# chansoopark98/Deep-Visual-SLAM

Measured on AMD Instinct MI355X. Metric: VO training-step frames/sec (3-frame 640x480 snippets), higher is better.
Workload: dtype f32; 1 GPU; configs[2]/[3]: full 4-scale photometric+smoothness loss, batch 12 per GPU, ResNet-18; per_gpu_batch=12, global_batch=12, num_scales=4, image=640x480, parallelism=dp1, streams=depth | pose | 2x weight-gradient, optimizer=fused Adam pass at lr 0: every step computes from the seeded weights, gpu_max_hw_queues=4

## Files before the change

deep-visual-slam_amd/csrc/conv_dma.h:

```cpp
#pragma once

__device__ __attribute__((aligned(16))) float g_dvs_zero_page[4] = {0.f, 0.f, 0.f, 0.f};

__device__ __forceinline__ void dma16(const float* gp, float* lds_wave_base) {
    __builtin_amdgcn_global_load_lds((const __attribute__((address_space(1))) void*)gp,
                                     (__attribute__((address_space(3))) void*)lds_wave_base, 16, 0, 0);
}

template <int TM, int TN>
__device__ __forceinline__ void mfma_stage_swz(const float* __restrict__ As, const float* __restrict__ Bs, int a_row0,
                                               int b_row0, int lane, f32x16 (&acc)[TM][TN]) {
    const int r = lane & 31, h = lane >> 5;
#pragma unroll
    for (int j = 0; j < BK / 8; ++j) {
        f32x4 a[TM], b[TN];
#pragma unroll
        for (int m = 0; m < TM; ++m) {
            int row = a_row0 + m * 32 + r;
            a[m] = *reinterpret_cast<const f32x4*>(As + row * BK + (((2 * j + h) ^ ((row >> 1) & 7)) << 2));
        }
#pragma unroll
        for (int n = 0; n < TN; ++n) {
            int row = b_row0 + n * 32 + r;
            b[n] = *reinterpret_cast<const f32x4*>(Bs + row * BK + (((2 * j + h) ^ ((row >> 1) & 7)) << 2));
        }
#pragma unroll
        for (int t = 0; t < 4; ++t)
#pragma unroll
            for (int m = 0; m < TM; ++m)
#pragma unroll
                for (int n = 0; n < TN; ++n)
                    acc[m][n] = __builtin_amdgcn_mfma_f32_32x32x2f32(a[m][t], b[n][t], acc[m][n], 0, 0, 0);
    }
}

template <int I, int N, class F>
__device__ __forceinline__ void static_for(F&& f) {
    if constexpr (I < N) {
        f(std::integral_constant<int, I>{});
        static_for<I + 1, N>(f);
    }
}

template <int BM, int BN, int WM, int WN, int MODE>
__global__ __launch_bounds__(NT) void conv_dma_kernel(FwdParams p) {
    constexpr int TM = BM / WM / 32, TN = BN / WN / 32;
    constexpr int A_INS = BM / 32, B_INS = BN / 32;
    constexpr int MAXTAP = 9;
    static_assert(WM * WN == 4 && TM >= 1 && TN >= 1, "4 waves");
    extern __shared__ __attribute__((aligned(16))) float smem[];
    float* As = smem;
    float* Bs = smem + 2 * BM * BK;

    ConvShape s = p.s;
    const int tid = threadIdx.x, lane = tid & 63;
    const int wave = __builtin_amdgcn_readfirstlane(tid >> 6);
    const int wm = wave / WN, wn = wave % WN;
    int bid_x, bid_y, bid_z, ks = 0;
    if (p.g.z > 1) {
        int lg = blockIdx.x;
        bid_x = lg % p.g.x;
        lg /= p.g.x;
        bid_y = lg % p.g.y;
        bid_z = lg / p.g.y;
    } else {
        const int tiles = p.g.x * p.g.y;
        int lg = blockIdx.x;
        if (p.ksplit > 1) {
            ks = lg % p.ksplit;
            lg /= p.ksplit;
        }
        lg = xcd_logical(lg, tiles, p.ksplit > 1 ? 0 : p.g.remap);
        bid_y = lg % p.g.y;
        bid_x = lg / p.g.y;
        bid_z = 0;
    }
    const int m0 = bid_x * BM, n0 = bid_y * BN;

    int Hr = s.Ho, Wr = s.Wo, rstep = 1, oy0 = 0, ox0 = 0, ky0 = 0, kx0 = 0;
    if (MODE == IN_DGRAD && s.stride == 2) {
        const int py = bid_z >> 1, px = bid_z & 1;
        oy0 = (py - s.pad) & 1;
        ox0 = (px - s.pad) & 1;
        Hr = (s.Ho - oy0 + 1) >> 1;
        Wr = (s.Wo - ox0 + 1) >> 1;
        rstep = 2;
        ky0 = py;
        kx0 = px;
        s.kh = py < s.kh ? (s.kh - py + 1) >> 1 : 0;
        s.kw = px < s.kw ? (s.kw - px + 1) >> 1 : 0;
        s.Ktot = s.kh * s.kw * s.Cin;
    }
    const int M = s.B * Hr * Wr;
    if (m0 >= M) return;
    const int ntap = s.kh * s.kw, nC = s.Cin / BK;
    const int c_per = (nC + p.ksplit - 1) / max(p.ksplit, 1);
    const int c_lo = p.ksplit > 1 ? ks * c_per : 0, c_hi = p.ksplit > 1 ? min(nC, c_lo + c_per) : nC;

    constexpr int NO_TAP = OOB_OFF;
    const int rsub = lane >> 3, slot = lane & 7;
    int toff[A_INS][MAXTAP];
    int toff2[(MODE == IN_UPCAT) ? A_INS : 1][MAXTAP];
    int r_b[A_INS], r_y[A_INS], r_x[A_INS], r_q[A_INS];
    bool r_ok[A_INS];
#pragma unroll
    for (int j = 0; j < A_INS; ++j) {
        const int row = (wave * A_INS + j) * 8 + rsub;
        r_q[j] = (slot ^ ((row >> 1) & 7)) << 2;
        int m = m0 + row;
        r_ok[j] = m < M;
        m = min(m, M - 1);
        const int b = m / (Hr * Wr), rem = m - b * (Hr * Wr);
        const int oy = rem / Wr, ox = rem - oy * Wr;
        r_b[j] = b;
        if (MODE == IN_DGRAD) {
            r_y[j] = oy * rstep + oy0 + s.pad;
            r_x[j] = ox * rstep + ox0 + s.pad;
        } else {
            r_y[j] = oy * s.stride - s.pad;
            r_x[j] = ox * s.stride - s.pad;
        }
    }
    int kc_tap[MAXTAP];
#pragma unroll
    for (int t = 0; t < MAXTAP; ++t) {
        kc_tap[t] = 0;
#pragma unroll
        for (int j = 0; j < A_INS; ++j) {
            toff[j][t] = NO_TAP;
            if (MODE == IN_UPCAT) toff2[j][t] = NO_TAP;
        }
        if (t < ntap) {
            const int tky = (t >= s.kw ? 1 : 0) + (t >= 2 * s.kw ? 1 : 0), tkx = t - tky * s.kw;
            kc_tap[t] = (MODE == IN_DGRAD) ? ((ky0 + rstep * tky) * p.s.kw + (kx0 + rstep * tkx)) * s.Cin : t * s.Cin;
#pragma unroll
            for (int j = 0; j < A_INS; ++j) {
                bool ok = r_ok[j];
                int off = 0, off2 = 0;
                if (MODE == IN_DGRAD) dgrad_tap_setup(p.s, r_b[j], r_y[j], r_x[j], ky0 + rstep * tky, kx0 + rstep * tkx, ok, off);
                else tap_setup<MODE>(s, p.t, r_b[j], r_y[j] + tky, r_x[j] + tkx, ok, off, off2);
                toff[j][t] = ok ? (off + r_q[j]) * 4 : NO_TAP;
                if (MODE == IN_UPCAT) toff2[j][t] = ok ? (off2 + p.t.C1 + r_q[j]) * 4 : NO_TAP;
            }
        }
    }
    int b_off[B_INS];
#pragma unroll
    for (int j = 0; j < B_INS; ++j) {
        const int row = (wave * B_INS + j) * 8 + rsub;
        const int n = n0 + row;
        b_off[j] = (n < s.Cout) ? (n * p.s.Ktot + ((slot ^ ((row >> 1) & 7)) << 2)) * 4 : NO_TAP;
    }
    const size_t x_elems = (MODE == IN_UPCAT) ? (size_t)s.B * (s.H >> 1) * (s.W >> 1) * p.t.C1 : (size_t)s.B * s.H * s.W * s.Cin;
    const __amdgpu_buffer_rsrc_t rx = dma_rsrc(p.x, x_elems * 4);
    const __amdgpu_buffer_rsrc_t rx2 = (MODE == IN_UPCAT && p.t.x2 != p.x)
                                           ? dma_rsrc(p.t.x2, (size_t)s.B * s.H * s.W * (s.Cin - p.t.C1) * 4) : rx;
    const __amdgpu_buffer_rsrc_t rw = dma_rsrc(p.w, (size_t)p.s.Cout * p.s.Ktot * 4);

    auto issue = [&](auto tc, int c, int buf) {
        constexpr int T = decltype(tc)::value;
        const int ci0 = c * BK;
        if (MODE == IN_UPCAT && ci0 >= p.t.C1) {
            const int soff = (ci0 - p.t.C1) * 4;
#pragma unroll
            for (int j = 0; j < A_INS; ++j) dma16_buf(rx2, toff2[j][T], soff, As + (buf * BM + (wave * A_INS + j) * 8) * BK);
        } else {
            const int soff = ci0 * 4;
#pragma unroll
            for (int j = 0; j < A_INS; ++j) dma16_buf(rx, toff[j][T], soff, As + (buf * BM + (wave * A_INS + j) * 8) * BK);
        }
        const int kc = (kc_tap[T] + ci0) * 4;
#pragma unroll
        for (int j = 0; j < B_INS; ++j) dma16_buf(rw, b_off[j], kc, Bs + (buf * BN + (wave * B_INS + j) * 8) * BK);
    };

    f32x16 acc[TM][TN];
#pragma unroll
    for (int m = 0; m < TM; ++m)
#pragma unroll
        for (int n = 0; n < TN; ++n)
#pragma unroll
            for (int i = 0; i < 16; ++i) acc[m][n][i] = 0.f;

    int buf = 0;
    auto compute_and_sync = [&]() {
        mfma_stage_swz<TM, TN>(As + buf * BM * BK, Bs + buf * BN * BK, wm * TM * 32, wn * TN * 32, lane, acc);
        asm volatile("s_waitcnt vmcnt(0)" ::: "memory");
        __syncthreads();
        buf ^= 1;
    };
    if (ntap > 0) {
        issue(std::integral_constant<int, 0>{}, c_lo, 0);
        asm volatile("s_waitcnt vmcnt(0)" ::: "memory");
        __syncthreads();
    }
    static_for<0, MAXTAP>([&](auto tc) {
        constexpr int T = decltype(tc)::value;
        if (T < ntap) {
#pragma unroll 1
            for (int c = c_lo; c + 1 < c_hi; ++c) {
                issue(tc, c + 1, buf ^ 1);
                compute_and_sync();
            }
            if constexpr (T + 1 < MAXTAP) {
                if (T + 1 < ntap) issue(std::integral_constant<int, T + 1>{}, c_lo, buf ^ 1);
            }
            compute_and_sync();
        }
    });
    int* rowtab = nullptr;
    if (MODE == IN_DGRAD && rstep == 2) {
        rowtab = reinterpret_cast<int*>(smem);
        fill_row_table<BM>(p, s, rowtab, m0, M, Hr, Wr, rstep, oy0, ox0);
    }
    conv_epilogue<TM, TN, MODE>(p, s, acc, m0, n0, wm, wn, lane, M, Hr, Wr, rstep, oy0, ox0, rowtab, BM);
}
```

deep-visual-slam_amd/csrc/conv_fwd.hip:

```cpp
#include "conv_common.h"

#include <cstdlib>
#include <type_traits>

namespace {
using namespace dvsconv;

struct FwdParams {
    const float* x;
    const float* w;
    const float* bias;
    float* y;
    float* stats;
    int stat_split;
    float* y2;
    int split_c1;
    int dbg_nobarrier;
    const float* zero_page;
    const float* res;
    int stat_mask, stat_stride;
    int work_m;
    int ksplit;
    Grid3 g;
    ConvShape s;
// ... 130 lines not shown
        for (int tn = 0; tn < TN; ++tn) {
            const int n = n0 + (wn * TN + tn) * 32 + ln;
#pragma unroll
            for (int tm = 0; tm < TM; ++tm) {
                const int mb = m0 + (wm * TM + tm) * 32 + 4 * lh;
#pragma unroll
                for (int i = 0; i < 16; ++i) {
                    const int m = mb + (i & 3) + 8 * (i >> 2);
                    if (m < M && n < s.Cout) atomicAdd(p.y + (size_t)m * s.Cout + n, acc[tm][tn][i]);
                }
            }
        }
    } else if (stats == 0) {
        if (p.res) conv_epilogue_body<TM, TN, MODE, 0, true, true>(p, s, acc, m0, n0, wm, wn, lane, M, rowtab, bm);
        else if (act) conv_epilogue_body<TM, TN, MODE, 0, true>(p, s, acc, m0, n0, wm, wn, lane, M, rowtab, bm);
        else conv_epilogue_body<TM, TN, MODE, 0, false>(p, s, acc, m0, n0, wm, wn, lane, M, rowtab, bm);
    } else if (stats == 1) {
        if (act) conv_epilogue_body<TM, TN, MODE, 1, true>(p, s, acc, m0, n0, wm, wn, lane, M, rowtab, bm);
        else conv_epilogue_body<TM, TN, MODE, 1, false>(p, s, acc, m0, n0, wm, wn, lane, M, rowtab, bm);
    } else {
        conv_epilogue_body<TM, TN, MODE, 2, true>(p, s, acc, m0, n0, wm, wn, lane, M, rowtab, bm);
    }
}

#include "conv_dma.h"

template <int BM, int BN, int WM, int WN, int MODE, bool FOLD, int NBUF, bool BF16 = false>
__global__ __launch_bounds__(NT) void conv_fwd_kernel(FwdParams p) {
    constexpr int TM = BM / WM / 32, TN = BN / WN / 32;
    constexpr int A_VECS = BM / 32, B_VECS = BN / 32;
    static_assert(WM * WN == 4 && TM >= 1 && TN >= 1, "4 waves");
    extern __shared__ __attribute__((aligned(16))) float smem[];
    float* As = smem;
    float* Bs = smem + NBUF * BM * LDK;
    __bf16* Ah = reinterpret_cast<__bf16*>(smem);
    __bf16* Bh = Ah + NBUF * BM * LDKH;

    ConvShape s = p.s;
    const int tid = threadIdx.x, lane = tid & 63, wave = tid >> 6;
    const int wm = wave / WN, wn = wave % WN;
    int bid_x, bid_y, bid_z;
    if (p.g.z > 1) {
        int lg = blockIdx.x;
        bid_x = lg % p.g.x;
        lg /= p.g.x;
        bid_y = lg % p.g.y;
        bid_z = lg / p.g.y;
    } else {
        int lg = xcd_logical(blockIdx.x, p.g.x * p.g.y, p.g.remap);
        bid_y = lg % p.g.y;
        bid_x = lg / p.g.y;
        bid_z = 0;
    }
    const int m0 = bid_x * BM, n0 = bid_y * BN;
    const int c4 = (tid & 7) * 4, r0 = tid >> 3;

    int Hr = s.Ho, Wr = s.Wo, rstep = 1, oy0 = 0, ox0 = 0, ky0 = 0, kx0 = 0, kw_full = s.kw;
    if (MODE == IN_DGRAD && s.stride == 2) {
        const int py = bid_z >> 1, px = bid_z & 1;
        oy0 = (py - s.pad) & 1;
        ox0 = (px - s.pad) & 1;
        Hr = (s.Ho - oy0 + 1) >> 1;
        Wr = (s.Wo - ox0 + 1) >> 1;
        rstep = 2;
        ky0 = py;
        kx0 = px;
        s.kh = py < s.kh ? (s.kh - py + 1) >> 1 : 0;
        s.kw = px < s.kw ? (s.kw - px + 1) >> 1 : 0;
        s.Ktot = s.kh * s.kw * s.Cin;
    }
    const int M = s.B * Hr * Wr;
    if (m0 >= M) return;

    int a_b[A_VECS], a_iy[A_VECS], a_ix[A_VECS];
    bool a_ok[A_VECS];
#pragma unroll
    for (int j = 0; j < A_VECS; ++j) {
        int m = m0 + r0 + 32 * j;
        a_ok[j] = m < M;
        m = min(m, M - 1);
        int b = m / (Hr * Wr), rem = m - b * (Hr * Wr);
        int oy = rem / Wr, ox = rem - oy * Wr;
        a_b[j] = b;
        if (MODE == IN_DGRAD) {
            a_iy[j] = oy * rstep + oy0 + s.pad;
            a_ix[j] = ox * rstep + ox0 + s.pad;
        } else {
            a_iy[j] = oy * s.stride - s.pad;
            a_ix[j] = ox * s.stride - s.pad;
        }
    }
    const float* b_ptr[B_VECS];
    bool b_ok[B_VECS];
#pragma unroll
    for (int j = 0; j < B_VECS; ++j) {
        int n = n0 + r0 + 32 * j;
        b_ok[j] = n < s.Cout;
        b_ptr[j] = p.w + (size_t)min(n, s.Cout - 1) * p.s.Ktot;
    }

    KPos kp;
    kp.init(c4, s);
    f32x4 ra[A_VECS], rb[B_VECS], ry[A_VECS], re[A_VECS], fsc, fsh;
    bool ra_ok[A_VECS], rb_ok;
    unsigned ra_mask[A_VECS];
    float psc = 1.f, psh = 0.f;
    int t_off[A_VECS], t_off2[A_VECS], cur_tap = -1;
    bool t_ok[A_VECS];
    auto load_stage = [&]() {
        const bool k_ok = kp.k < s.Ktot;
        int kc = min(kp.k, p.s.Ktot - 4);
        const int ky = ky0 + rstep * kp.ky, kx = kx0 + rstep * kp.kx;
        if (MODE == IN_DGRAD) kc = k_ok ? (ky * kw_full + kx) * s.Cin + kp.ci : 0;
        const int tap = ky * kw_full + kx;
        if (MODE != IN_PLANAR && tap != cur_tap) {
            cur_tap = tap;
#pragma unroll
            for (int j = 0; j < A_VECS; ++j) {
                bool ok = a_ok[j];
                if (MODE == IN_DGRAD) dgrad_tap_setup(p.s, a_b[j], a_iy[j], a_ix[j], ky, kx, ok, t_off[j]);
                else tap_setup<MODE>(s, p.t, a_b[j], a_iy[j] + kp.ky, a_ix[j] + kp.kx, ok, t_off[j], t_off2[j]);
                t_ok[j] = ok;
                if (p.dbg_nobarrier & 2) t_off[j] = t_off2[j] = 0;
            }
        }
#pragma unroll
        for (int j = 0; j < A_VECS; ++j) {
            if (MODE == IN_PLANAR) {
                int ci;
                ra[j] = gather_planar_raw(p.x, s, a_b[j], a_iy[j], a_ix[j], kc, a_ok[j] && k_ok, ra_mask[j], ci);
                if (FOLD && j == 0) {
                    psc = p.t.in_scale[ci];
                    psh = p.t.in_shift[ci];
                }
            } else if (MODE == IN_DGRAD) {
                ra[j] = *reinterpret_cast<const f32x4*>(p.x + (t_off[j] + kp.ci));
                if (p.t.dact) ry[j] = *reinterpret_cast<const f32x4*>(p.t.aux + (t_off[j] + kp.ci));
                re[j] = f32x4{0.f, 0.f, 0.f, 0.f};
                if (p.s.pad_mode == PAD_REFLECT)
                    re[j] = dgrad_reflect_extra(p.x, p.s, p.t, a_b[j], a_iy[j], a_ix[j], ky, kx, kp.ci, a_ok[j] && k_ok);
                ra_ok[j] = t_ok[j] && k_ok;
            } else {
                ra[j] = load_tap4<MODE>(p.x, p.t, t_off[j], t_off2[j], kp.ci);
                ra_ok[j] = t_ok[j] && k_ok;
            }
        }
        if (FOLD && MODE != IN_PLANAR) {
            fsc = *reinterpret_cast<const f32x4*>(p.t.in_scale + kp.ci);
            fsh = *reinterpret_cast<const f32x4*>(p.t.in_shift + kp.ci);
        }
#pragma unroll
        for (int j = 0; j < B_VECS; ++j) rb[j] = *reinterpret_cast<const f32x4*>(b_ptr[j] + kc);
        rb_ok = k_ok;
        if (MODE == IN_PLANAR) kp.k += BK;
        else kp.advance(s);
    };
    auto store_stage = [&](int buf) {
#pragma unroll
        for (int j = 0; j < A_VECS; ++j) {
            f32x4 v;
            if (MODE == IN_PLANAR) v = finalize_planar<FOLD>(ra[j], ra_mask[j], psc, psh);
            else if (MODE == IN_DGRAD) v = finalize_dgrad(ra[j], ry[j], re[j], ra_ok[j], p.t.dact);
            else v = finalize<FOLD>(ra[j], ra_ok[j], fsc, fsh, p.t.in_relu);
            if constexpr (BF16) *reinterpret_cast<bf16x4*>(Ah + (buf * BM + r0 + 32 * j) * LDKH + c4) = to_bf16(v);
            else *reinterpret_cast<f32x4*>(As + (buf * BM + r0 + 32 * j) * LDK + c4) = v;
        }
#pragma unroll
        for (int j = 0; j < B_VECS; ++j) {
            const bool ok = b_ok[j] && rb_ok;
            f32x4 v = rb[j];
#pragma unroll
            for (int e = 0; e < 4; ++e) v[e] = ok ? v[e] : 0.f;
            if constexpr (BF16) *reinterpret_cast<bf16x4*>(Bh + (buf * BN + r0 + 32 * j) * LDKH + c4) = to_bf16(v);
            else *reinterpret_cast<f32x4*>(Bs + (buf * BN + r0 + 32 * j) * LDK + c4) = v;
        }
    };

    f32x16 acc[TM][TN];
#pragma unroll
    for (int m = 0; m < TM; ++m)
#pragma unroll
        for (int n = 0; n < TN; ++n)
#pragma unroll
            for (int i = 0; i < 16; ++i) acc[m][n][i] = 0.f;

    const int KT = (s.Ktot + BK - 1) / BK;
    load_stage();
    store_stage(0);
    __syncthreads();
#pragma unroll 1
    for (int kt = 0; kt < KT; ++kt) {
        const int buf = (NBUF == 2) ? (kt & 1) : 0;
        const bool staged = !(p.dbg_nobarrier & 4);
        if (staged && kt + 1 < KT) load_stage();
        if constexpr (BF16) mfma_stage_bf16<TM, TN>(Ah + buf * BM * LDKH, Bh + buf * BN * LDKH, wm * TM * 32, wn * TN * 32, lane, acc);
        else mfma_stage<TM, TN>(As + buf * BM * LDK, Bs + buf * BN * LDK, wm * TM * 32, wn * TN * 32, lane, acc);
        if (NBUF == 1 && !(p.dbg_nobarrier & 1)) __syncthreads();
        if (staged && kt + 1 < KT) store_stage((NBUF == 2) ? (buf ^ 1) : 0);
        if (!(p.dbg_nobarrier & 1)) __syncthreads();
    }

    int* rowtab = nullptr;
    if (MODE == IN_DGRAD && (rstep == 2 || p.split_c1 > 0)) {
        rowtab = reinterpret_cast<int*>(smem);
        fill_row_table<BM>(p, s, rowtab, m0, M, Hr, Wr, rstep, oy0, ox0);
    }
    conv_epilogue<TM, TN, MODE>(p, s, acc, m0, n0, wm, wn, lane, M, Hr, Wr, rstep, oy0, ox0, rowtab, BM);
}

int conv_nbuf() {
    static int v = [] {
        const char* e = getenv("DVS_CONV_NBUF");
        return (e && e[0] == '2') ? 2 : 1;
    }();
    return v;
}

template <int BM, int BN, int WM, int WN, int MODE, bool FOLD, int NBUF, bool BF16 = false>
void launch_buf(const FwdParams& p, hipStream_t st, int slot);

template <int MODE, bool FOLD>
bool dma_eligible(const FwdParams& p) {
    static const bool enabled = [] { const char* e = getenv("DVS_CONV_DMA"); return !(e && e[0] == '0'); }();
    if (!enabled || FOLD || MODE == IN_PLANAR || (p.s.Cin % BK) != 0 || p.s.kh > 3 || p.s.kw > 3) return false;
    const double lim = 2147483648.0 / 4;
    if ((double)p.s.B * p.s.H * p.s.W * p.s.Cin >= lim || (double)p.s.Cout * p.s.Ktot >= lim) return false;
    if (MODE == IN_DGRAD) return p.t.dact == 0 && p.s.pad_mode == PAD_ZERO && p.split_c1 == 0;
    return true;
}

inline int xcd_remap_enabled() {
    static const int on = [] { const char* e = getenv("DVS_CONV_XCD"); return !(e && e[0] == '0') ? 1 : 0; }();
    return on;
}

__global__ __launch_bounds__(256) void splitk_finish_kernel(float* __restrict__ y, const float* __restrict__ bias,
                                                            const float* __restrict__ res, size_t nvec, int cout4, int act) {
    const size_t i = (size_t)blockIdx.x * 256 + threadIdx.x;
    if (i >= nvec) return;
    f32x4 v = reinterpret_cast<f32x4*>(y)[i];
    if (bias) v += reinterpret_cast<const f32x4*>(bias)[i % cout4];
    if (res) v += reinterpret_cast<const f32x4*>(res)[i];
#pragma unroll
    for (int e = 0; e < 4; ++e) v[e] = apply_act(v[e], act);
    reinterpret_cast<f32x4*>(y)[i] = v;
}

__global__ __launch_bounds__(256) void splitk_zero_kernel(float* __restrict__ y, size_t nvec) {
    const size_t i = (size_t)blockIdx.x * 256 + threadIdx.x;
    if (i < nvec) reinterpret_cast<f32x4*>(y)[i] = f32x4{0.f, 0.f, 0.f, 0.f};
}

template <int BM, int BN, int WM, int WN, int MODE>
void launch_dma(const FwdParams& p, hipStream_t st, int slot) {
    int M = p.s.B * p.s.Ho * p.s.Wo;
    dim3 grid((M + BM - 1) / BM, (p.s.Cout + BN - 1) / BN);
    if (MODE == IN_DGRAD && p.s.stride == 2) {
        int mc = p.s.B * ((p.s.Ho + 1) / 2) * ((p.s.Wo + 1) / 2);
        grid = dim3((mc + BM - 1) / BM, (p.s.Cout + BN - 1) / BN, 4);
    }
    size_t lds = (size_t)2 * (BM + BN) * BK * sizeof(float);
    auto kern = conv_dma_kernel<BM, BN, WM, WN, MODE>;
    static bool attr_set = false;
    if (!attr_set && lds > 64 * 1024 - 256) {
        (void)hipFuncSetAttribute(reinterpret_cast<const void*>(kern), hipFuncAttributeMaxDynamicSharedMemorySize, (int)lds);
        attr_set = true;
    }
    dvs::ProfScope prof(slot, st);
    const double eff = (MODE == IN_DGRAD) ? 1.0 / (p.s.stride * p.s.stride) : 1.0;
    prof.work(2.0 * (p.work_m ? p.work_m : M) * p.s.Cout * (double)p.s.Ktot * eff);
    FwdParams q = p;
    q.g = Grid3{(int)grid.x, (int)grid.y, (int)grid.z, xcd_remap_enabled()};
    q.ksplit = 1;
    if (MODE != IN_DGRAD || (p.s.stride == 1 && p.split_c1 == 0)) {
        static const bool splitk = [] { const char* e = getenv("DVS_CONV_SPLITK"); return !(e && e[0] == '0'); }();
        const int tiles = grid.x * grid.y, nC = p.s.Cin / BK;
        static const int sk_tiles = [] { const char* e = getenv("DVS_SPLITK_TILES"); return e ? atoi(e) : 320; }();
        static const int sk_target = [] { const char* e = getenv("DVS_SPLITK_TARGET"); return e ? atoi(e) : 0; }();
        if (splitk && !dvs::deterministic() && !p.stats && tiles < sk_tiles && nC >= 2 && (p.s.Cout & 3) == 0) {
            const int target = sk_target > 0 ? sk_target : (tiles < 200 ? 256 : 1024);
            int want = min(nC, (target + tiles - 1) / tiles);
            const int per = (nC + want - 1) / want;
            q.ksplit = (nC + per - 1) / per;
        }
    }
    static const float* zp = [] {
        void* d = nullptr;
        (void)hipGetSymbolAddress(&d, HIP_SYMBOL(g_dvs_zero_page));
        return static_cast<const float*>(d);
    }();
    q.zero_page = zp;
    if (q.ksplit > 1) {
        const size_t nvec = (size_t)M * p.s.Cout / 4;
        hipLaunchKernelGGL(splitk_zero_kernel, dim3((unsigned)((nvec + 255) / 256)), dim3(256), 0, st, p.y, nvec);
        hipLaunchKernelGGL(kern, dim3(grid.x * grid.y * q.ksplit), dim3(NT), lds, st, q);
        if (p.bias || p.res || p.act != ACT_NONE)
            hipLaunchKernelGGL(splitk_finish_kernel, dim3((unsigned)((nvec + 255) / 256)), dim3(256), 0, st, p.y, p.bias, p.res,
                               nvec, p.s.Cout / 4, p.act);
        return;
    }
    hipLaunchKernelGGL(kern, dim3(grid.x * grid.y * grid.z), dim3(NT), lds, st, q);
}

template <int BM, int BN, int WM, int WN, int MODE, bool FOLD>
void launch_cfg(const FwdParams& p0, hipStream_t st, int slot) {
    FwdParams p = p0;
    if constexpr (MODE == IN_PLANAR) {
        if (dvs::precision_bf16()) {
            p.dbg_nobarrier = 0;
            launch_buf<BM, BN, WM, WN, MODE, FOLD, 2, true>(p, st, slot);
            return;
        }
    }
    if constexpr (!FOLD && MODE != IN_PLANAR) {
        if (dvs::precision_bf16() && (p.s.Cin & 3) == 0) {
            p.dbg_nobarrier = 0;
            launch_buf<BM, BN, WM, WN, MODE, FOLD, 2, true>(p, st, slot);
            return;
        }
        if (dma_eligible<MODE, FOLD>(p)) {
            launch_dma<BM, BN, WM, WN, MODE>(p, st, slot);
            return;
        }
    }
    static const int nobar = dvs::experiment_flags("DVS_CONV_DEBUG_NOBARRIER");
    p.dbg_nobarrier = nobar;
    if (conv_nbuf() == 2) launch_buf<BM, BN, WM, WN, MODE, FOLD, 2>(p, st, slot);
    else launch_buf<BM, BN, WM, WN, MODE, FOLD, 1>(p, st, slot);
}

template <int BM, int BN, int WM, int WN, int MODE, bool FOLD, int NBUF, bool BF16>
void launch_buf(const FwdParams& p, hipStream_t st, int slot) {
    int M = p.s.B * p.s.Ho * p.s.Wo;
    dim3 grid((M + BM - 1) / BM, (p.s.Cout + BN - 1) / BN);
    if (MODE == IN_DGRAD && p.s.stride == 2) {
        int mc = p.s.B * ((p.s.Ho + 1) / 2) * ((p.s.Wo + 1) / 2);
        grid = dim3((mc + BM - 1) / BM, (p.s.Cout + BN - 1) / BN, 4);
    }
    size_t lds = BF16 ? (size_t)NBUF * (BM + BN) * LDKH * 2 : (size_t)NBUF * (BM + BN) * LDK * sizeof(float);
    if (BF16 && MODE == IN_DGRAD && lds < (size_t)2 * BM * sizeof(int)) lds = (size_t)2 * BM * sizeof(int);
    auto kern = conv_fwd_kernel<BM, BN, WM, WN, MODE, FOLD, NBUF, BF16>;
    static bool attr_set = false;
    if (!attr_set && lds > 64 * 1024) {
        (void)hipFuncSetAttribute(reinterpret_cast<const void*>(kern), hipFuncAttributeMaxDynamicSharedMemorySize, (int)lds);
        attr_set = true;
    }
    dvs::ProfScope prof(slot, st);
    const double k_real = (MODE == IN_PLANAR) ? (double)p.s.Cin * p.s.kh * p.s.kw : (double)p.s.Ktot;
    const double eff = (MODE == IN_DGRAD) ? 1.0 / (p.s.stride * p.s.stride) : 1.0;
    prof.work(2.0 * (p.work_m ? p.work_m : M) * p.s.Cout * k_real * eff);
    FwdParams q = p;
    q.g = Grid3{(int)grid.x, (int)grid.y, (int)grid.z, xcd_remap_enabled()};
    hipLaunchKernelGGL(kern, dim3(grid.x * grid.y * grid.z), dim3(NT), lds, st, q);
}

template <int MODE, bool FOLD>
void launch_mode(const FwdParams& p, hipStream_t st, int slot) {
    const ConvShape& s = p.s;
    const int M = s.B * s.Ho * s.Wo;
    static const bool small = [] { const char* e = getenv("DVS_CONV_TILE"); return e && e[0] == 's'; }();
    if constexpr (MODE == IN_DGRAD && !FOLD) {
        static const bool n96 = [] { const char* e = getenv("DVS_CONV_N96"); return !(e && e[0] == '0'); }();
        if (n96 && s.Cout == 96 && (dvs::precision_bf16() || !dma_eligible<MODE, FOLD>(p))) {
            FwdParams q = p;
            q.dbg_nobarrier = 0;
            if (dvs::precision_bf16()) launch_buf<128, 96, 4, 1, MODE, FOLD, 2, true>(q, st, slot);
            else if (conv_nbuf() == 2) launch_buf<128, 96, 4, 1, MODE, FOLD, 2>(q, st, slot);
            else launch_buf<128, 96, 4, 1, MODE, FOLD, 1>(q, st, slot);
            return;
        }
    }
    if (s.Cout > 64) {
        static const bool small_m = [] { const char* e = getenv("DVS_CONV_SMALLM"); return !(e && e[0] == '0'); }();
        const int t64 = ((M + 63) / 64) * ((s.Cout + 127) / 128);
        const int t128 = ((M + 127) / 128) * ((s.Cout + 127) / 128);
        const double rounds = t128 / 512.0, full = ceil(rounds);
        const bool tail_waste = rounds <= 3.2 && (full - rounds) / full > 0.2;
        const bool gemm_small = s.kh == 1 && s.kw == 1 && MODE != IN_DGRAD && t64 < 224;
        if (small_m && MODE != IN_DGRAD && ((p.stats && t64 < 160) || gemm_small)) launch_cfg<64, 64, 2, 2, MODE, FOLD>(p, st, slot);
        else if (small || t128 < 448 || tail_waste) launch_cfg<64, 128, 1, 4, MODE, FOLD>(p, st, slot);
        else launch_cfg<128, 128, 2, 2, MODE, FOLD>(p, st, slot);
    } else if (s.Cout > 32) {
        if (small) launch_cfg<64, 64, 2, 2, MODE, FOLD>(p, st, slot);
        else launch_cfg<128, 64, 2, 2, MODE, FOLD>(p, st, slot);
    } else {
        launch_cfg<128, 32, 4, 1, MODE, FOLD>(p, st, slot);
    }
}

__global__ __launch_bounds__(256) void pack_wt_kernel(const float* __restrict__ w, float* __restrict__ wt, int Cout,
                                                      int Cin, int T) {
    __shared__ float tile[32][33];
    const int tap = blockIdx.z, ci0 = blockIdx.x * 32, co0 = blockIdx.y * 32;
    const int tx = threadIdx.x & 31, ty = threadIdx.x >> 5;
#pragma unroll
    for (int j = 0; j < 4; ++j) {
        int co = co0 + ty + 8 * j, ci = ci0 + tx;
        tile[ty + 8 * j][tx] = (co < Cout && ci < Cin) ? w[((size_t)co * T + tap) * Cin + ci] : 0.f;
    }
    __syncthreads();
#pragma unroll
    for (int j = 0; j < 4; ++j) {
        int ci = ci0 + ty + 8 * j, co = co0 + tx;
        if (ci < Cin && co < Cout) wt[((size_t)ci * T + tap) * Cout + co] = tile[tx][ty + 8 * j];
    }
}

__global__ __launch_bounds__(256) void act_bwd_kernel(const float* __restrict__ dy, const float* __restrict__ y,
                                                      float* __restrict__ dz, size_t nvec, int act, float* __restrict__ dbias,
                                                      int C) {
    __shared__ f32x4 red[256];
    f32x4 bsum = {0.f, 0.f, 0.f, 0.f};
    const size_t stride = (size_t)gridDim.x * 256;
    for (size_t i = (size_t)blockIdx.x * 256 + threadIdx.x; i < nvec; i += stride) {
        f32x4 g = reinterpret_cast<const f32x4*>(dy)[i];
        const f32x4 v = reinterpret_cast<const f32x4*>(y)[i];
        if (act == ACT_ELU) {
#pragma unroll
            for (int e = 0; e < 4; ++e) g[e] = fmaf(g[e], fminf(v[e], 0.f), g[e]);
        } else {
#pragma unroll
            for (int e = 0; e < 4; ++e) g[e] *= act_grad_from_out(v[e], act);
        }
        reinterpret_cast<f32x4*>(dz)[i] = g;
        bsum += g;
    }
    if (dbias) {
        const int cv = C / 4;
        red[threadIdx.x] = bsum;
        __syncthreads();
        if ((int)threadIdx.x < cv) {
            for (int k = threadIdx.x + cv; k < 256; k += cv) bsum += red[k];
#pragma unroll
            for (int e = 0; e < 4; ++e) atomicAdd(dbias + threadIdx.x * 4 + e, bsum[e]);
        }
    }
}

__device__ __forceinline__ f32x4 folded_at(const float* __restrict__ G, int b, int y, int x, int c, int H, int W, int C) {
    const int Wp = W + 2;
    const float* base = G + ((size_t)b * (H + 2)) * Wp * C + c;
    auto at = [&](int py, int px) { return *reinterpret_cast<const f32x4*>(base + ((size_t)py * Wp + px) * C); };
    const int ey = (y == 1) ? 0 : ((y == H - 2) ? H + 1 : -1), ex = (x == 1) ? 0 : ((x == W - 2) ? W + 1 : -1);
    f32x4 v = at(y + 1, x + 1);
    if (ey >= 0) v += at(ey, x + 1);
    if (ex >= 0) v += at(y + 1, ex);
    if (ey >= 0 && ex >= 0) v += at(ey, ex);
    if (H == 3 && y == 1) v += at(H + 1, x + 1) + ((ex >= 0) ? at(H + 1, ex) : f32x4{0.f, 0.f, 0.f, 0.f});
    if (W == 3 && x == 1) v += at(y + 1, W + 1) + ((ey >= 0) ? at(ey, W + 1) : f32x4{0.f, 0.f, 0.f, 0.f});
    if (H == 3 && W == 3 && y == 1 && x == 1) v += at(H + 1, W + 1);
    return v;
}
__global__ __launch_bounds__(256) void reflect_fold_kernel(const float* __restrict__ G, float* __restrict__ dx,
                                                           float* __restrict__ dx_skip, int B, int H, int W, int C, int C1) {
    const int cv = C / 4;
    const size_t i = (size_t)blockIdx.x * 256 + threadIdx.x;
    if (C1 == 0) {
        if (i >= (size_t)B * H * W * cv) return;
        const int c = (int)(i % cv) * 4;
        size_t m = i / cv;
        const int x = (int)(m % W);
        m /= W;
        const int y = (int)(m % H), b = (int)(m / H);
        *reinterpret_cast<f32x4*>(dx + (((size_t)b * H + y) * W + x) * C + c) = folded_at(G, b, y, x, c, H, W, C);
        return;
    }
    const int H2 = H >> 1, W2 = W >> 1;
    if (i >= (size_t)B * H2 * W2 * cv) return;
    const int c = (int)(i % cv) * 4;
    size_t m = i / cv;
    const int x2 = (int)(m % W2);
    m /= W2;
    const int y2 = (int)(m % H2), b = (int)(m / H2);
    f32x4 v[4];
#pragma unroll
    for (int q = 0; q < 4; ++q) v[q] = folded_at(G, b, 2 * y2 + (q >> 1), 2 * x2 + (q & 1), c, H, W, C);
    if (c < C1) {
        *reinterpret_cast<f32x4*>(dx + (((size_t)b * H2 + y2) * W2 + x2) * C1 + c) = (v[0] + v[1]) + (v[2] + v[3]);
    } else {
        const int cs = C - C1;
#pragma unroll
        for (int q = 0; q < 4; ++q)
            *reinterpret_cast<f32x4*>(dx_skip + (((size_t)b * H + 2 * y2 + (q >> 1)) * W + 2 * x2 + (q & 1)) * cs + (c - C1)) = v[q];
    }
}

struct PackEntry {
    const float* w;
    float* wt;
    int Cout, Cin, T, wg_begin;
};
__global__ __launch_bounds__(256) void pack_wt_batch_kernel(const PackEntry* __restrict__ tab, int n) {
    __shared__ float tile[32][33];
    __shared__ int s_e;
    if (threadIdx.x == 0) {
        int e = 0;
        while (e + 1 < n && (int)blockIdx.x >= tab[e + 1].wg_begin) ++e;
        s_e = e;
    }
    __syncthreads();
    const PackEntry en = tab[s_e];
    const int tci = (en.Cin + 31) / 32, tco = (en.Cout + 31) / 32;
    int local = blockIdx.x - en.wg_begin;
    const int tap = local / (tci * tco);
    local -= tap * tci * tco;
    const int co0 = (local / tci) * 32, ci0 = (local % tci) * 32;
    const int tx = threadIdx.x & 31, ty = threadIdx.x >> 5;
#pragma unroll
    for (int j = 0; j < 4; ++j) {
        int co = co0 + ty + 8 * j, ci = ci0 + tx;
        tile[ty + 8 * j][tx] = (co < en.Cout && ci < en.Cin) ? en.w[((size_t)co * en.T + tap) * en.Cin + ci] : 0.f;
    }
    __syncthreads();
#pragma unroll
    for (int j = 0; j < 4; ++j) {
        int ci = ci0 + ty + 8 * j, co = co0 + tx;
        if (ci < en.Cin && co < en.Cout) en.wt[((size_t)ci * en.T + tap) * en.Cout + co] = tile[tx][ty + 8 * j];
    }
}

}

extern "C" {

int dvs_reflect_fold(const float* g_padded, float* dx, float* dx_skip, int B, int H, int W, int C, int C1, void* stream) {
    DVS_REQUIRE(g_padded && dx && B > 0 && H >= 3 && W >= 3 && C > 0 && (C & 3) == 0, "dvs_reflect_fold: bad argument");
    DVS_REQUIRE(C1 == 0 || ((C1 & 3) == 0 && C1 <= C && !((H | W) & 1) && (C1 == C || dx_skip)), "dvs_reflect_fold: bad split");
    const size_t n = (C1 == 0 ? (size_t)B * H * W : (size_t)B * (H / 2) * (W / 2)) * (C / 4);
    hipStream_t st = static_cast<hipStream_t>(stream);
    dvs::ProfScope prof(dvs::SLOT_CONV_DGRAD, st);
    hipLaunchKernelGGL(reflect_fold_kernel, dim3((unsigned)((n + 255) / 256)), dim3(256), 0, st, g_padded, dx, dx_skip, B, H, W, C, C1);
    return dvs::check_launch("dvs_reflect_fold");
}

int dvs_act_bwd(const float* dy, const float* y, float* dz, size_t n, int act, float* dbias, int C, void* stream) {
    DVS_REQUIRE(dy && y && dz && n > 0 && (n & 3) == 0 && act >= 0 && act <= 3, "dvs_act_bwd: bad argument");
    DVS_REQUIRE(!dbias || (C >= 4 && (C & 3) == 0 && C / 4 <= 256 && 256 % (C / 4) == 0 && n % C == 0),
                "dvs_act_bwd: the bias gradient needs C/4 to divide 256 (C=%d)", C);
    const size_t nvec = n / 4;
    size_t blocks = (nvec + 255) / 256;
    if (blocks > 512) blocks = 512;
    if (dbias) {
        size_t few = nvec / (256 * 32);
        few = few < 32 ? 32 : few;
        if (blocks > few) blocks = few;
    }
    hipStream_t st = static_cast<hipStream_t>(stream);
    dvs::ProfScope prof(dvs::SLOT_CONV_DGRAD, st);
    hipLaunchKernelGGL(act_bwd_kernel, dim3((unsigned)blocks), dim3(256), 0, st, dy, y, dz, nvec, act, dbias, C);
    return dvs::check_launch("dvs_act_bwd");
}

int dvs_conv2d_pack_wt_batch(const void* table, int n_entries, int total_workgroups, void* stream) {
    DVS_REQUIRE(table && n_entries > 0 && total_workgroups > 0, "dvs_conv2d_pack_wt_batch: bad argument");
    hipLaunchKernelGGL(pack_wt_batch_kernel, dim3(total_workgroups), dim3(256), 0, static_cast<hipStream_t>(stream),
                       static_cast<const PackEntry*>(table), n_entries);
    return dvs::check_launch("dvs_conv2d_pack_wt_batch");
}

int dvs_conv2d_pack_wt(const float* w, float* wt, int Cout, int Cin, int kh, int kw, void* stream) {
    DVS_REQUIRE(w && wt && Cout > 0 && Cin > 0 && kh > 0 && kw > 0, "dvs_conv2d_pack_wt: bad argument");
    dim3 grid((Cin + 31) / 32, (Cout + 31) / 32, kh * kw);
    hipLaunchKernelGGL(pack_wt_kernel, grid, dim3(256), 0, static_cast<hipStream_t>(stream), w, wt, Cout, Cin, kh * kw);
    return dvs::check_launch("dvs_conv2d_pack_wt");
}

int dvs_conv2d_dgrad(const float* dy, const float* wt, float* dx, const dvs_conv_desc* d, const float* y_out,
                     int dact, float* dx_skip, int C1, void* stream) {
    return dvs_conv2d_dgrad_res(dy, wt, dx, d, y_out, dact, dx_skip, C1, nullptr, stream);
}

int dvs_conv2d_dgrad_res(const float* dy, const float* wt, float* dx, const dvs_conv_desc* d, const float* y_out,
                         int dact, float* dx_skip, int C1, const float* residual, void* stream) {
    DVS_REQUIRE(dy && wt && dx && d, "dvs_conv2d_dgrad: null pointer");
    DVS_REQUIRE(!residual || (C1 == 0 && residual != dx), "dvs_conv2d_dgrad: a residual excludes the upsample+concat split and may not alias dx");
    DVS_REQUIRE(C1 == 0 || (d->stride == 1 && (d->H & 1) == 0 && (d->W & 1) == 0 && C1 <= d->Cin &&
                            (C1 == d->Cin || dx_skip != nullptr)),
                "dvs_conv2d_dgrad: bad upsample+concat split");
    DVS_REQUIRE(d->stride == 1 || d->stride == 2, "dvs_conv2d_dgrad: stride %d (1 or 2 supported)", d->stride);
    DVS_REQUIRE((d->Cout & 3) == 0 && (d->Cin & 3) == 0, "dvs_conv2d_dgrad: channel counts must be multiples of 4");
    DVS_REQUIRE(d->pad_mode == PAD_ZERO || (d->pad_mode == 2 && d->pad == 0 && d->stride == 1 && d->H > 2 && d->W > 2 && !dact && !C1) ||
                    (d->pad_mode == PAD_REFLECT && d->pad == 1 && d->kh == 3 && d->kw == 3 && d->stride == 1 && d->H >= 2 && d->W >= 2),
                "dvs_conv2d_dgrad: reflect mode is ReflectionPad2d(1) + 3x3 stride 1 only; pad_mode 2 = pre-padded input, pad 0");
    DVS_REQUIRE(!dact || y_out, "dvs_conv2d_dgrad: activation gradient needs the forward output");
    DVS_REQUIRE((double)d->B * d->H * d->W * (d->Cin > d->Cout ? d->Cin : d->Cout) < 2147483648.0,
                "dvs_conv2d_dgrad: tensors must have fewer than 2^31 elements (32-bit gather offsets)");
    FwdParams p{};
    p.x = dy; p.w = wt; p.y = dx;
    p.stat_split = 0x7fffffff;
    ConvShape& s = p.s;
    int Ho = (d->H + 2 * d->pad - d->kh) / d->stride + 1, Wo = (d->W + 2 * d->pad - d->kw) / d->stride + 1;
    s.B = d->B;
    s.Ho = d->H; s.Wo = d->W; s.Cout = d->Cin;
    s.H = Ho; s.W = Wo; s.Cin = d->Cout;
    s.kh = d->kh; s.kw = d->kw; s.stride = d->stride; s.pad = d->pad; s.pad_mode = d->pad_mode;
    if (d->pad_mode == 2) {
        s.pad_mode = PAD_ZERO;
        p.work_m = d->B * (d->H - 2) * (d->W - 2);
    }
    s.Ktot = d->kh * d->kw * d->Cout;
    p.t.aux = y_out;
    p.t.dact = dact;
    p.y2 = dx_skip;
    p.split_c1 = C1;
    p.res = residual;
    hipStream_t st = static_cast<hipStream_t>(stream);
    if (!residual && d->pad_mode == PAD_REFLECT && d->kh == 3 && d->kw == 3 && d->stride == 1 && d->pad == 1 &&
        thin_dgrad(dy, wt, dx, y_out, dact, d->B, d->H, d->W, d->Cin, d->Cout, C1, dx_skip, st))
        return dvs::check_launch("dvs_conv2d_dgrad");
    launch_mode<IN_DGRAD, false>(p, st, dvs::SLOT_CONV_DGRAD);
    return dvs::check_launch("dvs_conv2d_dgrad");
}

int dvs_conv2d_fwd(const float* x, const float* w, const float* bias, float* y, const dvs_conv_desc* d,
                   const dvs_conv_fusion* f, void* stream) {
    DVS_REQUIRE(x && w && y && d, "dvs_conv2d_fwd: null pointer");
    DVS_REQUIRE(d->B > 0 && d->H > 0 && d->W > 0 && d->Cin > 0 && d->Cout > 0 && d->kh > 0 && d->kw > 0 &&
                    d->stride > 0 && d->pad >= 0,
                "dvs_conv2d_fwd: bad descriptor");
    FwdParams p{};
    p.x = x; p.w = w; p.bias = bias; p.y = y;
    p.stat_split = 0x7fffffff;
    ConvShape& s = p.s;
    s.B = d->B; s.H = d->H; s.W = d->W; s.Cin = d->Cin; s.Cout = d->Cout;
    s.kh = d->kh; s.kw = d->kw; s.stride = d->stride; s.pad = d->pad; s.pad_mode = d->pad_mode;
    s.Ho = (d->H + 2 * d->pad - d->kh) / d->stride + 1;
    s.Wo = (d->W + 2 * d->pad - d->kw) / d->stride + 1;
    DVS_REQUIRE(s.Ho > 0 && s.Wo > 0, "dvs_conv2d_fwd: empty output");
    DVS_REQUIRE((double)d->B * d->H * d->W * d->Cin < 2147483648.0 && (double)d->B * s.Ho * s.Wo * d->Cout < 2147483648.0,
                "dvs_conv2d_fwd: tensors must have fewer than 2^31 elements (32-bit gather offsets)");
    DVS_REQUIRE(d->pad_mode == PAD_ZERO || (d->pad < d->H && d->pad < d->W), "dvs_conv2d_fwd: reflect pad too large");
    int planar = 0;
    if (f) {
        p.t.x2 = f->x2; p.t.C1 = f->C1; p.t.in_scale = f->in_scale; p.t.in_shift = f->in_shift;
        p.t.in_relu = f->in_relu; planar = f->nchw_planar;
        p.act = f->act; p.stats = f->stats; p.res = f->residual;
        DVS_REQUIRE(f->act >= 0 && f->act <= ACT_GELU, "dvs_conv2d_fwd: unknown activation %d", f->act);
        DVS_REQUIRE(!(f->residual && f->stats), "dvs_conv2d_fwd: residual and stats are exclusive (inference vs training)");
        DVS_REQUIRE(f->stat_groups >= 0 && f->stat_groups <= 2 && (f->stat_groups != 2 || (d->B % 2) == 0),
                    "dvs_conv2d_fwd: stat_groups is 0, 1 or 2 (2 needs an even batch)");
        p.stat_split = (f->stat_groups == 2) ? (d->B / 2) * s.Ho * s.Wo : 0x7fffffff;
        if (f->stats && f->stat_slots > 1) {
            DVS_REQUIRE(f->stat_slots <= 64 && (f->stat_slots & (f->stat_slots - 1)) == 0 && !f->nchw_planar,
                        "dvs_conv2d_fwd: stat_slots must be a power of two <= 64 (NHWC input only)");
            p.stat_mask = f->stat_slots - 1;
            p.stat_stride = (f->stat_groups == 2 ? 2 : 1) * 2 * d->Cout;
        }
        DVS_REQUIRE(!(f->x2) || (f->C1 > 0 && (d->H & 1) == 0 && (d->W & 1) == 0 &&
                                 ((f->C1 == d->Cin && (f->C1 & 3) == 0) || (f->C1 < d->Cin && (f->C1 % BK) == 0))),
                    "dvs_conv2d_fwd: upsample+concat needs C1 %% 32 == 0 (or C1 == Cin) and even H, W");
        DVS_REQUIRE(!(f->x2 && planar), "dvs_conv2d_fwd: planar input cannot be concatenated");
        DVS_REQUIRE((f->in_scale == nullptr) == (f->in_shift == nullptr), "dvs_conv2d_fwd: in_scale/in_shift come together");
    }
    if (planar) {
        DVS_REQUIRE(d->kw <= 8 && d->pad_mode == PAD_ZERO, "dvs_conv2d_fwd: planar input supports kw <= 8, zero padding");
        s.Ktot = d->Cin * d->kh * 8;
    } else {
        DVS_REQUIRE((d->Cin & 3) == 0, "dvs_conv2d_fwd: NHWC input needs Cin %% 4 == 0 (got %d)", d->Cin);
        s.Ktot = d->kh * d->kw * d->Cin;
    }
    hipStream_t st = static_cast<hipStream_t>(stream);
    const bool fold = p.t.in_scale != nullptr;
    static const bool stem16 = [] { const char* e = getenv("DVS_BF16_STEM"); return e && e[0] == '1'; }();
// ... 20 lines not shown
```

Before: 1537 frames/s.

## Merge stride-2 dgrad parity classes into one kernel with shared input tiles

Adds a dedicated stride-2 data-gradient conv kernel that handles all four output parity classes in a single launch. Each loaded gradient tile is reused across the taps of every class, with separate accumulators per class. Stores go through a per-row pixel table held in LDS. Previously the z-grid launched the parity classes as separate blocks that each reloaded the input. The new kernel raises register pressure (four accumulator sets for 3x3) and serializes the classes inside one block, trading parallelism for input reuse.

```diff
diff --git a/deep-visual-slam_amd/csrc/conv_dma.h b/deep-visual-slam_amd/csrc/conv_dma.h
--- a/deep-visual-slam_amd/csrc/conv_dma.h
+++ b/deep-visual-slam_amd/csrc/conv_dma.h
@@ -215,3 +215,177 @@
     }
     conv_epilogue<TM, TN, MODE>(p, s, acc, m0, n0, wm, wn, lane, M, Hr, Wr, rstep, oy0, ox0, rowtab, BM);
 }
+
+template <bool K3>
+struct S2Map {
+    static constexpr int pad = K3 ? 1 : 0;
+    static constexpr int first_shift = K3 ? 0 : 3;
+    static constexpr int nacc = K3 ? 4 : 1;
+    static constexpr int sy(int S) { return 1 - (S >> 1); }
+    static constexpr int sx(int S) { return 1 - (S & 1); }
+    static constexpr int ntap(int S) { return K3 ? (sy(S) ? 1 : 2) * (sx(S) ? 1 : 2) : (S == 3 ? 1 : 0); }
+    static constexpr int a(int S, int U) { return K3 ? 1 - U / (sx(S) ? 1 : 2) : 0; }
+    static constexpr int b(int S, int U) { return K3 ? 1 - U % (sx(S) ? 1 : 2) : 0; }
+    static constexpr int ky(int S, int U) { return a(S, U) + pad - 2 * sy(S); }
+    static constexpr int kx(int S, int U) { return b(S, U) + pad - 2 * sx(S); }
+    static constexpr int acc(int S, int U) { return K3 ? a(S, U) * 2 + b(S, U) : 0; }
+};
+
+template <int BM, int BN, int WM, int WN, bool K3>
+__global__ __launch_bounds__(NT, 2) void conv_dgrad_s2m_kernel(FwdParams p) {
+    using Map = S2Map<K3>;
+    constexpr int TM = BM / WM / 32, TN = BN / WN / 32;
+    constexpr int A_INS = BM / 32, B_INS = BN / 32;
+    constexpr int NACC = Map::nacc, S0 = Map::first_shift;
+    static_assert(WM * WN == 4 && TM >= 1 && TN >= 1 && BM <= NT, "4 waves; one thread per row fills the pixel table");
+    extern __shared__ __attribute__((aligned(16))) float smem[];
+    float* As = smem;
+    float* Bs = smem + 2 * BM * BK;
+
+    const ConvShape& s = p.s;
+    const int tid = threadIdx.x, lane = tid & 63;
+    const int wave = __builtin_amdgcn_readfirstlane(tid >> 6);
+    const int wm = wave / WN, wn = wave % WN;
+    const int lg = xcd_logical(blockIdx.x, p.g.x * p.g.y, p.g.remap);
+    const int m0 = (lg / p.g.y) * BM, n0 = (lg % p.g.y) * BN;
+    const int Hb = (s.Ho + 1) >> 1, Wb = (s.Wo + 1) >> 1, M = s.B * Hb * Wb;
+    if (m0 >= M) return;
+    const int nC = s.Cin / BK;
+
+    constexpr int NO_TAP = OOB_OFF;
+    const int rsub = lane >> 3, slot = lane & 7;
+    int toff[A_INS][4];
+#pragma unroll
+    for (int j = 0; j < A_INS; ++j) {
+        const int row = (wave * A_INS + j) * 8 + rsub;
+        const int q = (slot ^ ((row >> 1) & 7)) << 2;
+        int m = m0 + row;
+        const bool ok = m < M;
+        m = min(m, M - 1);
+        const int b = m / (Hb * Wb), rem = m - b * (Hb * Wb);
+        const int by = rem / Wb, bx = rem - by * Wb;
+#pragma unroll
+        for (int S = 0; S < 4; ++S) {
+            const int ty = by + Map::sy(S), tx = bx + Map::sx(S);
+            const bool in = ok && S >= S0 && ty < s.H && tx < s.W;
+            toff[j][S] = in ? (((b * s.H + ty) * s.W + tx) * s.Cin + q) * 4 : NO_TAP;
+        }
+    }
+    int b_off[B_INS];
+#pragma unroll
+    for (int j = 0; j < B_INS; ++j) {
+        const int row = (wave * B_INS + j) * 8 + rsub;
+        const int n = n0 + row;
+        b_off[j] = (n < s.Cout) ? (n * s.Ktot + ((slot ^ ((row >> 1) & 7)) << 2)) * 4 : NO_TAP;
+    }
+    const __amdgpu_buffer_rsrc_t rx = dma_rsrc(p.x, (size_t)s.B * s.H * s.W * s.Cin * 4);
+    const __amdgpu_buffer_rsrc_t rw = dma_rsrc(p.w, (size_t)s.Cout * s.Ktot * 4);
+    const size_t dx_bytes = (size_t)s.B * s.Ho * s.Wo * s.Cout * 4;
+    const __amdgpu_buffer_rsrc_t ry = dma_rsrc(p.y, dx_bytes);
+    const __amdgpu_buffer_rsrc_t rr = dma_rsrc(p.res ? p.res : p.y, dx_bytes);
+
+    auto issue_a = [&](auto sc, int c, int buf) {
+        constexpr int S = decltype(sc)::value;
+        const int soff = c * BK * 4;
+#pragma unroll
+        for (int j = 0; j < A_INS; ++j) dma16_buf(rx, toff[j][S], soff, As + (buf * BM + (wave * A_INS + j) * 8) * BK);
+    };
+    auto issue_b = [&](auto sc, auto uc, int c, int buf) {
+        constexpr int S = decltype(sc)::value, U = decltype(uc)::value;
+        const int kc = ((Map::ky(S, U) * s.kw + Map::kx(S, U)) * s.Cin + c * BK) * 4;
+#pragma unroll
+        for (int j = 0; j < B_INS; ++j) dma16_buf(rw, b_off[j], kc, Bs + (buf * BN + (wave * B_INS + j) * 8) * BK);
+    };
+
+    f32x16 acc[NACC][TM][TN];
+#pragma unroll
+    for (int k = 0; k < NACC; ++k)
+#pragma unroll
+        for (int m = 0; m < TM; ++m)
+#pragma unroll
+            for (int n = 0; n < TN; ++n)
+#pragma unroll
+                for (int i = 0; i < 16; ++i) acc[k][m][n][i] = 0.f;
+
+    int abuf = 0, bbuf = 0;
+    using I0 = std::integral_constant<int, 0>;
+    issue_a(std::integral_constant<int, S0>{}, 0, 0);
+    issue_b(std::integral_constant<int, S0>{}, I0{}, 0, 0);
+    asm volatile("s_waitcnt vmcnt(0)" ::: "memory");
+    __syncthreads();
+    static_for<S0, 4>([&](auto sc) {
+        constexpr int S = decltype(sc)::value;
+        constexpr int NU = Map::ntap(S);
+#pragma unroll 1
+        for (int c = 0; c < nC; ++c) {
+            static_for<0, NU>([&](auto uc) {
+                constexpr int U = decltype(uc)::value;
+                if constexpr (U + 1 < NU) {
+                    issue_b(sc, std::integral_constant<int, U + 1>{}, c, bbuf ^ 1);
+                } else {
+                    if (c + 1 < nC) {
+                        issue_a(sc, c + 1, abuf ^ 1);
+                        issue_b(sc, I0{}, c + 1, bbuf ^ 1);
+                    } else if constexpr (S + 1 < 4) {
+                        issue_a(std::integral_constant<int, S + 1>{}, 0, abuf ^ 1);
+                        issue_b(std::integral_constant<int, S + 1>{}, I0{}, 0, bbuf ^ 1);
+                    }
+                }
+                mfma_stage_swz<TM, TN>(As + abuf * BM * BK, Bs + bbuf * BN * BK, wm * TM * 32, wn * TN * 32, lane,
+                                       acc[Map::acc(S, U)]);
+                asm volatile("s_waitcnt vmcnt(0)" ::: "memory");
+                __syncthreads();
+                bbuf ^= 1;
+            });
+            abuf ^= 1;
+        }
+    });
+
+    int* tab = reinterpret_cast<int*>(smem);
+    if (tid < BM) {
+        const int m = m0 + tid;
+        const int mc = min(m, M - 1);
+        const int b = mc / (Hb * Wb), rem = mc - b * (Hb * Wb);
+        const int by = rem / Wb, bx = rem - by * Wb;
+        const int off = ((b * s.Ho + 2 * by) * s.Wo + 2 * bx) * s.Cout * 4, dx1 = s.Cout * 4, dy1 = s.Wo * s.Cout * 4;
+        const bool ok = m < M, y1 = 2 * by + 1 < s.Ho, x1 = 2 * bx + 1 < s.Wo;
+        tab[tid] = ok ? off : NO_TAP;
+        tab[BM + tid] = (ok && x1) ? off + dx1 : NO_TAP;
+        tab[2 * BM + tid] = (ok && y1) ? off + dy1 : NO_TAP;
+        tab[3 * BM + tid] = (ok && y1 && x1) ? off + dy1 + dx1 : NO_TAP;
+    }
+    __syncthreads();
+    const int ln = lane & 31, lh = lane >> 5;
+    auto store_all = [&](auto resc) {
+        constexpr bool RES = decltype(resc)::value;
+        static_for<0, 4>([&](auto cc) {
+            constexpr int CLS = decltype(cc)::value;
+#pragma unroll
+            for (int tn = 0; tn < TN; ++tn) {
+                const int n = n0 + (wn * TN + tn) * 32 + ln;
+                const int noff = n < s.Cout ? n * 4 : NO_TAP;
+#pragma unroll
+                for (int tm = 0; tm < TM; ++tm) {
+                    const int rb = (wm * TM + tm) * 32 + 4 * lh;
+                    int off[16];
+#pragma unroll
+                    for (int i = 0; i < 16; ++i) off[i] = tab[CLS * BM + rb + (i & 3) + 8 * (i >> 2)] + noff;
+                    float rres[RES ? 16 : 1];
+                    if constexpr (RES) {
+#pragma unroll
+                        for (int i = 0; i < 16; ++i) rres[i] = __builtin_bit_cast(float, __builtin_amdgcn_raw_buffer_load_b32(rr, off[i], 0, 0));
+                    }
+#pragma unroll
+                    for (int i = 0; i < 16; ++i) {
+                        float v = 0.f;
+                        if constexpr (K3 || CLS == 0) v = acc[K3 ? CLS : 0][tm][tn][i];
+                        if constexpr (RES) v = v + rres[i];
+                        __builtin_amdgcn_raw_buffer_store_b32(__builtin_bit_cast(unsigned, v), ry, off[i], 0, 0);
+                    }
+                }
+            }
+        });
+    };
+    if (p.res) store_all(std::true_type{});
+    else store_all(std::false_type{});
+}
diff --git a/deep-visual-slam_amd/csrc/conv_fwd.hip b/deep-visual-slam_amd/csrc/conv_fwd.hip
--- a/deep-visual-slam_amd/csrc/conv_fwd.hip
+++ b/deep-visual-slam_amd/csrc/conv_fwd.hip
@@ -456,6 +456,33 @@
     hipLaunchKernelGGL(kern, dim3(grid.x * grid.y * grid.z), dim3(NT), lds, st, q);
 }
 
+bool dgrad_s2_merged(const FwdParams& p) {
+    static const bool enabled = [] { const char* e = getenv("DVS_DGRAD_S2_MERGED"); return !(e && e[0] == '0'); }();
+    const ConvShape& s = p.s;
+    if (!enabled || s.stride != 2 || dvs::precision_bf16() || !dma_eligible<IN_DGRAD, false>(p)) return false;
+    const bool k3 = s.kh == 3 && s.kw == 3 && s.pad == 1, k1 = s.kh == 1 && s.kw == 1 && s.pad == 0;
+    static const int min_tiles = [] { const char* e = getenv("DVS_DGRAD_S2_MIN_TILES"); return e ? atoi(e) : 256; }();
+    const int mb = s.B * ((s.Ho + 1) / 2) * ((s.Wo + 1) / 2);
+    if (k3 && ((mb + 63) / 64) * ((s.Cout + 63) / 64) < min_tiles) return false;
+    return (k3 || k1) && s.H <= (s.Ho + 1) / 2 && s.W <= (s.Wo + 1) / 2 && (double)s.B * s.Ho * s.Wo * s.Cout < 2147483648.0 / 4;
+}
+
+template <int BM, int BN, int WM, int WN>
+void launch_dgrad_s2m(const FwdParams& p, hipStream_t st, int slot) {
+    const int M = p.s.B * p.s.Ho * p.s.Wo;
+    const int mb = p.s.B * ((p.s.Ho + 1) / 2) * ((p.s.Wo + 1) / 2);
+    dim3 grid((mb + BM - 1) / BM, (p.s.Cout + BN - 1) / BN);
+    const size_t lds = (size_t)2 * (BM + BN) * BK * sizeof(float);
+    static_assert(2 * (BM + BN) * BK >= 4 * BM && 2 * (BM + BN) * BK * sizeof(float) <= 64 * 1024, "pixel table fits, default LDS limit");
+    dvs::ProfScope prof(slot, st);
+    prof.work(2.0 * (p.work_m ? p.work_m : M) * p.s.Cout * (double)p.s.Ktot * 0.25);
+    FwdParams q = p;
+    q.g = Grid3{(int)grid.x, (int)grid.y, 1, xcd_remap_enabled()};
+    q.ksplit = 1;
+    if (p.s.kh == 3) hipLaunchKernelGGL((conv_dgrad_s2m_kernel<BM, BN, WM, WN, true>), dim3(grid.x * grid.y), dim3(NT), lds, st, q);
+    else hipLaunchKernelGGL((conv_dgrad_s2m_kernel<BM, BN, WM, WN, false>), dim3(grid.x * grid.y), dim3(NT), lds, st, q);
+}
+
 template <int BM, int BN, int WM, int WN, int MODE, bool FOLD>
 void launch_cfg(const FwdParams& p0, hipStream_t st, int slot) {
     FwdParams p = p0;
@@ -513,6 +540,18 @@
     const ConvShape& s = p.s;
     const int M = s.B * s.Ho * s.Wo;
     static const bool small = [] { const char* e = getenv("DVS_CONV_TILE"); return e && e[0] == 's'; }();
+    if constexpr (MODE == IN_DGRAD && !FOLD) {
+        if (dgrad_s2_merged(p)) {
+            static const int small_below = [] { const char* e = getenv("DVS_DGRAD_S2_SMALL_BELOW"); return e ? atoi(e) : 256; }();
+            const int mb = s.B * ((s.Ho + 1) / 2) * ((s.Wo + 1) / 2);
+            const int big = s.Cout > 64 ? ((mb + 63) / 64) * ((s.Cout + 127) / 128) : ((mb + 127) / 128) * ((s.Cout + 63) / 64);
+            if (s.Cout > 32 && big < small_below) launch_dgrad_s2m<64, 64, 2, 2>(p, st, slot);
+            else if (s.Cout > 64) launch_dgrad_s2m<64, 128, 1, 4>(p, st, slot);
+            else if (s.Cout > 32) launch_dgrad_s2m<128, 64, 2, 2>(p, st, slot);
+            else launch_dgrad_s2m<128, 32, 4, 1>(p, st, slot);
+            return;
+        }
+    }
     if constexpr (MODE == IN_DGRAD && !FOLD) {
         static const bool n96 = [] { const char* e = getenv("DVS_CONV_N96"); return !(e && e[0] == '0'); }();
         if (n96 && s.Cout == 96 && (dvs::precision_bf16() || !dma_eligible<MODE, FOLD>(p))) {
```

Result: no change. 1544 frames/s (median of 6 runs) (+0.5%).
